# swesterfeld/audiowmark

Hardware: AMD Instinct MI355X
Metric: audio seconds watermarked+decoded per wall-second (xRT), 44.1 kHz stereo (higher is better)
Workload: dtype f32; 1 GPU; 60 min stereo 44.1 kHz white noise per GPU resident in HBM, add+get incl. payload decode, payload 0123456789abcdef0011223344556677, strength 10; parallelism=1 GPU, patterns=108, payload_matches=104, ranks_seen=1

## Files before the change

audiowmark_amd/csrc/hip/kernels.hip:

```cpp
#include "kernels.hh"
#include "awm_fft.hip.h"
#include <cstdlib>
#include <algorithm>
#include <type_traits>

namespace awmk {

constexpr int NB = 81;
constexpr int MIN_BAND = 20;
constexpr int WAVES = 4;

typedef const int __attribute__ ((address_space (4))) *const_int_ptr;

__device__ __forceinline__ void
load_shared_tables (const DevTables& t, float2 *s_tw, float *s_win, float2 *s_twb)
{
  fft512_load_twiddles (t.tw512, s_tw);
  for (int i = threadIdx.x; i < 1024; i += blockDim.x)
    s_win[i] = t.window[i];
  if (s_twb)
    for (int i = threadIdx.x; i < NB; i += blockDim.x)
      s_twb[i] = t.tw1024[MIN_BAND + i];
}

// ... 2900 lines not shown
  const int R = a.table.rows_per_bit;
  const_int_ptr tab = (const_int_ptr) (a.table.packed + (size_t) bit * R * 64);

  float umag = 0.f, dmag = 0.f;
  int n = 0;
  for (int r = 0; r < R; r++)
    {
      const_int_ptr tr = tab + r * 64;
      const long long row = tr[60];
      const bool present = have ? have[row * a.have_row_stride] != 0 : true;
      if (have && !__any (present))
        continue;
      const float *p = db + row * a.row_stride;
      float uv[30], dv[30];
#pragma unroll
      for (int i = 0; i < 30; i++)
        {
          uv[i] = p[tr[i] * a.band_stride];
          dv[i] = p[tr[30 + i] * a.band_stride];
        }
      if (present)
        {
#pragma unroll
          for (int i = 0; i < 30; i++)
            {
              umag = __fadd_rn (umag, uv[i]);
              dmag = __fadd_rn (dmag, dv[i]);
            }
          n++;
        }
    }
  s_u[bit][lane] = umag;
  s_d[bit][lane] = dmag;
  s_n[bit][lane] = n;
  __syncthreads();
  if (bit == 0 && active)
    {
      double q = 0;
      int total = 0;
      for (int b = 0; b < 6; b++)
        {
          const float um = s_u[b][lane], dm = s_d[b][lane];
          float raw;
          if (um == 0 || dm == 0)
            raw = 0;
          else if (um < dm)
            raw = __fsub_rn (1.f, __fdiv_rn (um, dm));
          else
            raw = __fsub_rn (__fdiv_rn (dm, um), 1.f);
          const double rb = (b & 1) ? double (raw) : -double (raw);
          q += rb * s_n[b][lane];
          total += s_n[b][lane];
        }
      if (total)
        q /= total;
      q = q / a.min_delta / 2.9;
      a.quality[plane * a.q_stride + cand] = q;
    }
}

hipError_t
launch_sync_scan (hipStream_t st, const SyncScanArgs& a)
{
  if (a.n_lanes <= 0 || a.n_planes <= 0)
    return hipSuccess;
  SyncScanArgs b = a;
  long long done = 0;
  while (done < a.n_planes)
    {
      const long long n = (a.n_planes - done) > 65535 ? 65535 : (a.n_planes - done);
      b.db = a.db + done * a.plane_stride;
      b.have = a.have ? a.have + done * a.have_plane_stride : nullptr;
      b.lane_count = a.lane_count ? a.lane_count + done : nullptr;
      b.quality = a.quality + done * a.q_stride;
      const long long per_xcd = ((a.n_lanes + 63) / 64 + 7) / 8;
      const dim3 grid (unsigned (per_xcd * 8), unsigned (n));
      hipLaunchKernelGGL (sync_scan_kernel, grid, dim3 (64, 6), 0, st, b);
      hipError_t e = hipGetLastError();
      if (e != hipSuccess)
        return e;
      done += n;
    }
  return hipSuccess;
}

template<bool HAVE> __global__ void __launch_bounds__ (64)
sync_scan_gathered_kernel (GatheredScanArgs a)
{
  const int lane = threadIdx.x;
  const long long plane = blockIdx.y;
  const int count = a.lane_count[plane];
  int chain, cand;
  if (int (blockIdx.x) < a.regular_waves)
    {
      chain = blockIdx.x % 12;
      cand = (blockIdx.x / 12) * 64 + lane;
    }
  else
    {
      chain = lane / a.tail_lanes;
      cand = a.tail_first + lane % a.tail_lanes;
    }
  const bool active = chain < 12 && cand < count;
  if (!__any (active))
    return;
  if (!active)
    chain = 0, cand = 0;
  const int bit = chain >> 1, down = chain & 1;
  const int R = a.rows_per_bit;
  const int ld = a.ld;
  const bool from_tail = a.tail && cand >= ld;
  const long long step = from_tail ? 1 : ld;
  const float *p = from_tail ? a.tail + plane * a.tail_plane_stride + ((long long) bit * R * 60 + down * 30)
                             : a.db + plane * a.plane_stride + ((long long) bit * R * 60 + down * 30) * ld + cand;
  const int hld = a.have_ld ? a.have_ld : ld;
  const char *hv = HAVE ? a.have + plane * a.have_plane_stride + (long long) bit * R * hld + cand : nullptr;

  float mag = 0.f;
  int n = 0;
  auto issue = [&] (int r, float (&v)[30], bool& present) {
    const float *q = p + (long long) r * 60 * step;
    present = HAVE ? hv[r * hld] != 0 : true;
    if (HAVE && !__any (present))
      return;
#pragma unroll
    for (int i = 0; i < 30; i++)
      v[i] = q[i * step];
  };
  auto accumulate = [&] (const float (&v)[30], bool present) {
    if (present)
      {
#pragma unroll
        for (int i = 0; i < 30; i++)
          mag = __fadd_rn (mag, v[i]);
        n++;
      }
  };
  float v[3][30];
  bool pr[3] = { false, false, false };
  const int last = R - 1;
  int r = 0;
  if (R > 0)
    {
#pragma unroll
      for (int k = 0; k < 2; k++)
        {
          issue (k < last ? k : last, v[k], pr[k]);
          __builtin_amdgcn_sched_barrier (0);
        }
      for (; r + 3 <= R; r += 3)
        {
#pragma unroll
          for (int k = 0; k < 3; k++)
            {
              const int nx = r + k + 2;
              issue (nx < last ? nx : last, v[(k + 2) % 3], pr[(k + 2) % 3]);
              __builtin_amdgcn_sched_barrier (0);
              accumulate (v[k], pr[k]);
              __builtin_amdgcn_sched_barrier (0);
            }
        }
#pragma unroll
      for (int k = 0; k < 2; k++)
        if (r + k < R)
          accumulate (v[k], pr[k]);
    }
  if (active)
    {
      a.chain_mag[(plane * 12 + chain) * 128 + cand] = mag;
      if (!down)
        a.chain_n[(plane * 6 + bit) * 128 + cand] = n;
    }
}

__global__ void __launch_bounds__ (64)
sync_quality_kernel (GatheredScanArgs a)
{
  const long long plane = blockIdx.y;
  const int cand = blockIdx.x * 64 + threadIdx.x;
  if (cand >= a.lane_count[plane])
    return;
  double q = 0;
  int total = 0;
  for (int b = 0; b < 6; b++)
    {
      const float um = a.chain_mag[(plane * 12 + 2 * b) * 128 + cand], dm = a.chain_mag[(plane * 12 + 2 * b + 1) * 128 + cand];
      const int n = a.chain_n[(plane * 6 + b) * 128 + cand];
      float raw;
      if (um == 0 || dm == 0)
        raw = 0;
      else if (um < dm)
        raw = __fsub_rn (1.f, __fdiv_rn (um, dm));
      else
        raw = __fsub_rn (__fdiv_rn (dm, um), 1.f);
      const double rb = (b & 1) ? double (raw) : -double (raw);
      q += rb * n;
      total += n;
    }
  if (total)
    q /= total;
  q = q / a.min_delta / 2.9;
  a.quality[plane * a.q_stride + cand] = q;
}

hipError_t
launch_sync_scan_gathered (hipStream_t st, const GatheredScanArgs& a0)
{
  if (a0.n_lanes <= 0 || a0.n_planes <= 0)
    return hipSuccess;
  if (!a0.lane_count || a0.n_planes > 65535 || a0.n_lanes > 128 || !a0.chain_mag || !a0.chain_n)
    return hipErrorInvalidValue;
  GatheredScanArgs a = a0;
  const int full = a.n_lanes / 64, rem = a.n_lanes % 64;
  const bool tail = rem > 0 && rem * 12 <= 64;
  a.regular_waves = 12 * (tail || rem == 0 ? full : full + 1);
  a.tail_first = 64 * full;
  a.tail_lanes = tail ? rem : 1;
  const dim3 grid (unsigned (a.regular_waves + (tail ? 1 : 0)), unsigned (a.n_planes));
  if (a.have)
    hipLaunchKernelGGL (sync_scan_gathered_kernel<true>, grid, dim3 (64), 0, st, a);
  else
    hipLaunchKernelGGL (sync_scan_gathered_kernel<false>, grid, dim3 (64), 0, st, a);
  hipLaunchKernelGGL (sync_quality_kernel, dim3 (unsigned ((a.n_lanes + 63) / 64), unsigned (a.n_planes)), dim3 (64), 0, st, a);
  return hipGetLastError();
}

__global__ void __launch_bounds__ (256)
local_mean_kernel (const double *q, long long q_stride, long long S, double *raw_sorted, double *local_mean)
{
  const long long p = (long long) blockIdx.x * blockDim.x + threadIdx.x;
  const long long n_scores = 4 * S;
  if (p >= n_scores)
    return;
  q += (long long) blockIdx.y * 4 * q_stride;
  raw_sorted += (long long) blockIdx.y * n_scores;
  local_mean += (long long) blockIdx.y * n_scores;
  double avg = 0;
  int n = 0;
  for (int j = -20; j <= 20; j++)
    {
      if (j > -4 && j < 4)
        continue;
      const long long idx = p + j;
      if (idx >= 0 && idx < n_scores)
        {
          avg += q[(idx & 3) * q_stride + (idx >> 2)];
          n++;
        }
    }
  if (n > 0)
    avg /= n;
  raw_sorted[p] = q[(p & 3) * q_stride + (p >> 2)];
  local_mean[p] = avg;
}

hipError_t
launch_local_mean (hipStream_t st, const double *q, long long q_stride, long long n_start_frames, double *raw_sorted, double *local_mean,
                   int n_slices)
{
  const long long n = 4 * n_start_frames;
  if (n <= 0 || n_slices <= 0)
    return hipSuccess;
  hipLaunchKernelGGL (local_mean_kernel, dim3 (unsigned ((n + 255) / 256), unsigned (n_slices)), dim3 (256), 0, st, q, q_stride, n_start_frames,
                      raw_sorted, local_mean);
  return hipGetLastError();
}

__global__ void __launch_bounds__ (128)
soft_bits_kernel (SoftBitsArgs a)
{
  const long long blk = blockIdx.y;
  const int bit = blockIdx.x * blockDim.x + threadIdx.x;
  const int n_bits = a.n_data_frames / a.frames_per_bit;
  if (bit >= n_bits)
    return;
  const float *db = a.db + blk * a.block_stride;
  const int C = a.n_channels;
  const long long mix0 = a.block_slice ? (long long) a.block_slice[blk] * a.n_data_frames * 30 : 0;
  const int16_t *mix_frame = a.mix_frame + mix0;
  const uint8_t *mix_up = a.mix_up + mix0, *mix_down = a.mix_down + mix0;
  double umag = 0, dmag = 0;
  for (int f = bit * a.frames_per_bit; f < (bit + 1) * a.frames_per_bit; f++)
    for (int ch = 0; ch < C; ch++)
      {
        const float *plane = db + (long long) ch * NB * a.ld;
        for (int j = 0; j < 30; j++)
          {
            const int b = f * 30 + j;
            const int frame = mix_frame[b];
            const int next = frame + 1 < a.block_frames ? frame + 1 : frame - 1;
            const int prev = frame - 1 >= 0 ? frame - 1 : frame + 1;
            const float *pu = plane + (long long) (mix_up[b] - MIN_BAND) * a.ld;
            const float *pd = plane + (long long) (mix_down[b] - MIN_BAND) * a.ld;
            umag += pu[frame];
            umag -= double (__fadd_rn (pu[prev], pu[next])) * 0.5;
            dmag += pd[frame];
            dmag -= double (__fadd_rn (pd[prev], pd[next])) * 0.5;
          }
      }
  a.out[blk * n_bits + bit] = float (umag - dmag);
}

constexpr int SB_WAVES = 4;
constexpr int SB_BPW = 4;
constexpr int SB_MAX_ITEMS = 256;

__global__ void __launch_bounds__ (64 * SB_WAVES)
soft_bits_wave_kernel (SoftBitsArgs a, int groups_per_block)
{
  extern __shared__ __attribute__ ((aligned (16))) float4 s_item_dyn[];
  const int lane = threadIdx.x & 63, wave = threadIdx.x >> 6;
  const long long slot = blockIdx.x >> 3;
  const long long blk = (slot / groups_per_block) * 8 + (blockIdx.x & 7);
  const int group = int (slot % groups_per_block);
  if (blk >= a.n_blocks)
    return;
  const int n_bits = a.n_data_frames / a.frames_per_bit;
  const int bit0 = (group * SB_WAVES + wave) * SB_BPW;
  if (bit0 >= n_bits)
    return;
  const float *db = a.db + blk * a.block_stride;
  const int C = a.n_channels;
  const long long mix0 = a.block_slice ? (long long) a.block_slice[blk] * a.n_data_frames * 30 : 0;
  const int16_t *mix_frame = a.mix_frame + mix0;
  const uint8_t *mix_up = a.mix_up + mix0, *mix_down = a.mix_down + mix0;
  const int n_items = a.frames_per_bit * C * 30;
  float4 *items = s_item_dyn + (size_t) wave * SB_BPW * n_items;
  const int n_here = min (SB_BPW, n_bits - bit0);
  int live_lo = 0, live_hi = 0x7fffffff;
  if (a.stream_range)
    {
      const long long sl = a.range_index[blk];
      const long long first = a.stream_range[2 * sl], last = a.stream_range[2 * sl + 1];
      live_lo = a.block_frames;
      live_hi = -1;
      if (first >= 0)
        {
          const long long base = a.block_base[blk];
          const long long lo_num = (first + C - 1) / C - 1024 - base, hi_num = last / C - base;
          const long long lo = lo_num <= 0 ? 0 : (lo_num + 1023) / 1024, hi = hi_num < 0 ? -1 : hi_num / 1024;
          live_lo = int (lo < a.block_frames ? lo : a.block_frames);
          live_hi = int (hi < a.block_frames ? hi : a.block_frames - 1);
        }
    }
  const float zero_db = db_from_complex (make_float2 (0.f, 0.f));
  for (int i = lane; i < n_items; i += 64)
#pragma unroll
  for (int q = 0; q < SB_BPW; q++)
    {
      const int e = q * n_items + i;
      const int bit = bit0 + min (q, n_here - 1);
      const int fi = i / (C * 30), ch = (i / 30) % C, j = i % 30;
      const int b = (bit * a.frames_per_bit + fi) * 30 + j;
      const int frame = mix_frame[b];
      const int next = frame + 1 < a.block_frames ? frame + 1 : frame - 1;
      const int prev = frame - 1 >= 0 ? frame - 1 : frame + 1;
      if (max (frame, max (prev, next)) < live_lo || min (frame, min (prev, next)) > live_hi)
        {
          items[e] = make_float4 (zero_db, __fadd_rn (zero_db, zero_db), zero_db, __fadd_rn (zero_db, zero_db));
          continue;
        }
      const float *plane = db + (long long) ch * NB * a.ld;
      const float *pu = plane + (long long) (mix_up[b] - MIN_BAND) * a.ld;
      const float *pd = plane + (long long) (mix_down[b] - MIN_BAND) * a.ld;
      items[e] = make_float4 (pu[frame], __fadd_rn (pu[prev], pu[next]), pd[frame], __fadd_rn (pd[prev], pd[next]));
    }
  wave_sync();
  if (lane < n_here)
    {
      const float4 *mine = items + lane * n_items;
      double umag = 0, dmag = 0;
      for (int i = 0; i < n_items; i++)
        {
          const float4 t = mine[i];
          umag = __dadd_rn (umag, double (t.x));
          umag = __dsub_rn (umag, __dmul_rn (double (t.y), 0.5));
          dmag = __dadd_rn (dmag, double (t.z));
          dmag = __dsub_rn (dmag, __dmul_rn (double (t.w), 0.5));
        }
      a.out[blk * n_bits + bit0 + lane] = float (__dsub_rn (umag, dmag));
    }
}

int g_soft_bits_generic = 0;
extern "C" void awm_debug_set_soft_bits_generic (int on) { g_soft_bits_generic = on; }

hipError_t
launch_soft_bits (hipStream_t st, const SoftBitsArgs& a)
{
  if (a.n_blocks <= 0)
    return hipSuccess;
  const int n_bits = a.n_data_frames / a.frames_per_bit;
  if (!g_soft_bits_generic && a.frames_per_bit * a.n_channels * 30 <= SB_MAX_ITEMS)
    {
      const int groups = (n_bits + SB_WAVES * SB_BPW - 1) / (SB_WAVES * SB_BPW);
      const long long rounds = (a.n_blocks + 7) / 8;
      const long long wgs = rounds * groups * 8;
      const size_t lds = size_t (SB_WAVES) * SB_BPW * (a.frames_per_bit * a.n_channels * 30) * sizeof (float4);
      if (wgs < (1LL << 31))
        {
          hipLaunchKernelGGL (soft_bits_wave_kernel, dim3 (unsigned (wgs)), dim3 (64 * SB_WAVES), lds, st, a, groups);
          return hipGetLastError();
        }
    }
  const dim3 grid (unsigned ((n_bits + 127) / 128), unsigned (a.n_blocks));
  hipLaunchKernelGGL (soft_bits_kernel, grid, dim3 (128), 0, st, a);
  return hipGetLastError();
}

__global__ void __launch_bounds__ (256)
nonzero_range_kernel (const float *data, long long n_values, unsigned long long *result)
{
  const long long stride = (long long) gridDim.x * blockDim.x;
  unsigned long long first = ~0ULL, last = 0;
  for (long long i = (long long) blockIdx.x * blockDim.x + threadIdx.x; i < n_values; i += stride)
    if (data[i] != 0.f)
      {
        if ((unsigned long long) i < first) first = i;
        if ((unsigned long long) i + 1 > last) last = i + 1;
      }
  for (int o = 32; o > 0; o >>= 1)
    {
      const unsigned long long f = __shfl_xor (first, o), l = __shfl_xor (last, o);
      first = f < first ? f : first;
      last = l > last ? l : last;
    }
  __shared__ unsigned long long s_first[4], s_last[4];
  if ((threadIdx.x & 63) == 0)
    {
      s_first[threadIdx.x >> 6] = first;
      s_last[threadIdx.x >> 6] = last;
    }
  __syncthreads();
  if (threadIdx.x == 0)
    {
      for (int w = 1; w < 4; w++)
        {
          first = s_first[w] < first ? s_first[w] : first;
          last = s_last[w] > last ? s_last[w] : last;
        }
      if (first != ~0ULL)
        {
          atomicMin (result, first);
          atomicMax (result + 1, last);
        }
    }
}

__global__ void __launch_bounds__ (256)
soft_prep_kernel (SoftPrepArgs a)
{
  __shared__ __attribute__ ((aligned (16))) float s_v[1728];
  __shared__ double s_mean;
  const SoftJobDev job = a.jobs[blockIdx.x];
  const int2 *src = a.src + job.src_off;
  const int nb = a.n_bits;
  const int *inv_order = a.inv_order + job.order_off;
  if (job.len > 1728)
    return;
  if (job.mode == 0)
    {
      const float *raw = a.raw + (long long) src[0].x * nb;
      for (int k = threadIdx.x; k < nb; k += 256)
        s_v[k] = raw[inv_order[k]];
    }
  else if (job.mode == 1)
    {
      for (int s = 0; s < job.n_src; s++)
        {
          const float *raw = a.raw + (long long) src[s].x * nb;
          const int half = src[s].y;
          for (int k = threadIdx.x; k < nb; k += 256)
            s_v[2 * k + half] = raw[inv_order[k]];
        }
    }
  else
    {
      const float div0 = float (job.norm0 > 1 ? job.norm0 : 1), div1 = float (job.norm1 > 1 ? job.norm1 : 1);
      for (int k = threadIdx.x; k < nb; k += 256)
        {
          const int i = inv_order[k];
          float acc0 = 0.f, acc1 = 0.f;
          int s = 0;
          for (; s + 8 <= job.n_src; s += 8)
            {
              float v[8];
              int half[8];
#pragma unroll
              for (int u = 0; u < 8; u++)
                {
                  const int2 sp = src[s + u];
                  v[u] = a.raw[(long long) sp.x * nb + i];
                  half[u] = sp.y;
                }
#pragma unroll
              for (int u = 0; u < 8; u++)
                {
                  if (half[u])
                    acc1 = __fadd_rn (acc1, v[u]);
                  else
                    acc0 = __fadd_rn (acc0, v[u]);
                }
            }
          for (; s < job.n_src; s++)
            {
              const float v = a.raw[(long long) src[s].x * nb + i];
              if (src[s].y)
                acc1 = __fadd_rn (acc1, v);
              else
                acc0 = __fadd_rn (acc0, v);
            }
          s_v[2 * k] = __fdiv_rn (acc0, div0);
          s_v[2 * k + 1] = __fdiv_rn (acc1, div1);
        }
    }
  __syncthreads();
  float *out = a.out + job.out_off;
  if (a.hard)
    {
      for (int k = threadIdx.x; k < job.len; k += 256)
        out[k] = s_v[k] > 0 ? 1.f : 0.f;
      return;
    }
  if (threadIdx.x == 0)
    {
      double mean = 0;
      int k = 0;
      for (; k + 32 <= job.len; k += 32)
        {
          float4 q[8];
#pragma unroll
          for (int i = 0; i < 8; i++)
            q[i] = reinterpret_cast<const float4 *> (s_v + k)[i];
#pragma unroll
          for (int i = 0; i < 8; i++)
            {
              mean = __dadd_rn (mean, double (fabsf (q[i].x)));
              mean = __dadd_rn (mean, double (fabsf (q[i].y)));
              mean = __dadd_rn (mean, double (fabsf (q[i].z)));
              mean = __dadd_rn (mean, double (fabsf (q[i].w)));
            }
        }
      for (; k < job.len; k++)
        mean = __dadd_rn (mean, double (fabsf (s_v[k])));
      s_mean = __ddiv_rn (mean, double (job.len));
    }
  __syncthreads();
  const double mean = s_mean;
  for (int k = threadIdx.x; k < job.len; k += 256)
    out[k] = float (__dmul_rn (0.5, __dadd_rn (__ddiv_rn (double (s_v[k]), mean), 1.0)));
}

hipError_t
launch_soft_prep (hipStream_t st, const SoftPrepArgs& a)
{
  if (a.n_jobs <= 0)
    return hipSuccess;
  hipLaunchKernelGGL (soft_prep_kernel, dim3 (unsigned (a.n_jobs)), dim3 (256), 0, st, a);
  return hipGetLastError();
}

hipError_t
launch_nonzero_range (hipStream_t st, const float *data, long long n_values, unsigned long long *result)
{
  hipError_t e = hipMemsetAsync (result, 0xff, sizeof (unsigned long long), st);
  if (e == hipSuccess)
    e = hipMemsetAsync (result + 1, 0, sizeof (unsigned long long), st);
  if (e != hipSuccess || n_values <= 0)
    return e;
  hipLaunchKernelGGL (nonzero_range_kernel, dim3 (1024), dim3 (256), 0, st, data, n_values, result);
  return hipGetLastError();
}

__global__ void __launch_bounds__ (256)
clip_pad_kernel (const ClipSrc *src, float *dst, long long slice_values, long long margin_values, unsigned long long *range)
{
  const ClipSrc c = src[blockIdx.y];
  float4 *out = reinterpret_cast<float4 *> (dst + (long long) blockIdx.y * slice_values);
  const long long slice0 = (long long) blockIdx.y * slice_values;
  const long long stride = (long long) gridDim.x * blockDim.x;
  unsigned long long first = ~0ULL, last = 0;
  long long q_lo = (c.pad_start - margin_values) / 4, q_hi = (c.pad_start + c.n_values + margin_values + 3) / 4;
  q_lo = q_lo < 0 ? 0 : q_lo;
  q_hi = q_hi > slice_values / 4 ? slice_values / 4 : q_hi;
  for (long long q = q_lo + (long long) blockIdx.x * blockDim.x + threadIdx.x; q < q_hi; q += stride)
    {
      const long long k = 4 * q - c.pad_start;
      float v[4] = { 0.f, 0.f, 0.f, 0.f };
      if (k > -4 && k < c.n_values)
        {
#pragma unroll
          for (int j = 0; j < 4; j++)
            if (k + j >= 0 && k + j < c.n_values)
              v[j] = c.data[k + j];
#pragma unroll
          for (int j = 0; j < 4; j++)
            if (v[j] != 0.f)
              {
                const unsigned long long at = (unsigned long long) (slice0 + 4 * q + j);
                first = at < first ? at : first;
                last = at + 1 > last ? at + 1 : last;
              }
        }
      out[q] = make_float4 (v[0], v[1], v[2], v[3]);
    }
  for (int o = 32; o > 0; o >>= 1)
    {
      const unsigned long long f = __shfl_xor (first, o), l = __shfl_xor (last, o);
      first = f < first ? f : first;
      last = l > last ? l : last;
    }
  __shared__ unsigned long long s_first[4], s_last[4];
  if ((threadIdx.x & 63) == 0)
    {
      s_first[threadIdx.x >> 6] = first;
      s_last[threadIdx.x >> 6] = last;
    }
  __syncthreads();
  if (threadIdx.x == 0)
    {
      for (int w = 1; w < 4; w++)
        {
          first = s_first[w] < first ? s_first[w] : first;
          last = s_last[w] > last ? s_last[w] : last;
        }
      if (first != ~0ULL)
        {
          atomicMin (range + 2 * blockIdx.y, first);
          atomicMax (range + 2 * blockIdx.y + 1, last);
        }
    }
}

__global__ void
clip_range_init_kernel (unsigned long long *range, int n_clips)
{
  const int i = blockIdx.x * blockDim.x + threadIdx.x;
  if (i < n_clips)
    {
      range[2 * i] = ~0ULL;
      range[2 * i + 1] = 0;
    }
}

int g_clip_poison = 0;
extern "C" void awm_debug_set_clip_poison (int on) { g_clip_poison = on; }

hipError_t
launch_clip_pad (hipStream_t st, const ClipSrc *src, int n_clips, float *dst, long long slice_values, long long margin_values, long long *range)
{
  if (n_clips <= 0 || slice_values <= 0)
    return hipSuccess;
  if (slice_values % 4 || margin_values < 0 || (reinterpret_cast<uintptr_t> (dst) & 15))
    return hipErrorInvalidValue;
  if (g_clip_poison)
    if (hipError_t e = hipMemsetAsync (dst, 0xff, size_t (n_clips) * size_t (slice_values) * sizeof (float), st))
      return e;
  auto *r = reinterpret_cast<unsigned long long *> (range);
  hipLaunchKernelGGL (clip_range_init_kernel, dim3 (unsigned ((n_clips + 255) / 256)), dim3 (256), 0, st, r, n_clips);
  hipLaunchKernelGGL (clip_pad_kernel, dim3 (128, unsigned (n_clips)), dim3 (256), 0, st, src, dst, slice_values, margin_values, r);
  return hipGetLastError();
}

constexpr int SEG_RUN = 2048;
__global__ void __launch_bounds__ (256)
segment_copy_kernel (const SegmentCopy *copies)
{
  const SegmentCopy c = copies[blockIdx.y];
  const long long n_zero = c.zeros / 2, n_total = n_zero + c.n_values / 2;
  const long long base = (long long) blockIdx.x * SEG_RUN;
  if (c.n_values <= 0 || base >= n_total)
    return;
  const float2 *src = reinterpret_cast<const float2 *> (c.src);
  float2 *dst = reinterpret_cast<float2 *> (c.dst);
  constexpr int U = SEG_RUN / 256;
  float2 v[U];
#pragma unroll
  for (int j = 0; j < U; j++)
    {
      const long long q = base + threadIdx.x + 256 * j;
      v[j] = q >= n_zero && q < n_total ? src[q - n_zero] : make_float2 (0.f, 0.f);
    }
#pragma unroll
  for (int j = 0; j < U; j++)
    {
      const long long q = base + threadIdx.x + 256 * j;
      if (q < n_total)
        dst[q] = v[j];
    }
}

hipError_t
launch_segment_copy (hipStream_t st, const SegmentCopy *copies_dev, int n_copies, long long max_values)
{
  if (n_copies <= 0 || max_values <= 0)
    return hipSuccess;
  const long long max_pieces = (max_values + 1) / 2;
  hipLaunchKernelGGL (segment_copy_kernel, dim3 (unsigned ((max_pieces + SEG_RUN - 1) / SEG_RUN), unsigned (n_copies)), dim3 (256), 0, st, copies_dev);
  return hipGetLastError();
}

// ... 355 lines not shown
```

Before: 748,700 xRT.

## Pipeline soft-bit gathers with wave-specialized double-buffered LDS slices

Restructures the soft-bits kernel so that one wave accumulates the double-precision sums for 16 bits while the other three waves gather the next frame/channel slice into a double-buffered, padded LDS tile. The gather loads a contiguous 3-float run per band, replacing three scalar loads, and batches several gathers per iteration to raise memory-level parallelism. It also shrinks LDS from a per-wave item array to two small slices, which may raise occupancy. In exchange it adds a block-wide barrier per slice and serialises the accumulation onto a single wave, so throughput depends on whether the gather or the FP64 accumulation dominates.

```diff
diff --git a/audiowmark_amd/csrc/hip/kernels.hip b/audiowmark_amd/csrc/hip/kernels.hip
--- a/audiowmark_amd/csrc/hip/kernels.hip
+++ b/audiowmark_amd/csrc/hip/kernels.hip
@@ -3226,8 +3226,13 @@
 }
 
 constexpr int SB_WAVES = 4;
-constexpr int SB_BPW = 4;
+constexpr int SB_BITS = 16;
+constexpr int SB_ROW = SB_BITS + 1;
+constexpr int SB_GATHER_DEPTH = 3;
 constexpr int SB_MAX_ITEMS = 256;
+
+typedef float SbRun __attribute__ ((ext_vector_type (3), aligned (4)));
+static __device__ __forceinline__ float sb_pick (SbRun r, int i) { return i == 0 ? r.x : i == 1 ? r.y : r.z; }
 
 __global__ void __launch_bounds__ (64 * SB_WAVES)
 soft_bits_wave_kernel (SoftBitsArgs a, int groups_per_block)
@@ -3240,17 +3245,13 @@
   if (blk >= a.n_blocks)
     return;
   const int n_bits = a.n_data_frames / a.frames_per_bit;
-  const int bit0 = (group * SB_WAVES + wave) * SB_BPW;
-  if (bit0 >= n_bits)
-    return;
+  const int bit0 = group * SB_BITS;
+  const int n_here = min (SB_BITS, n_bits - bit0);
   const float *db = a.db + blk * a.block_stride;
   const int C = a.n_channels;
   const long long mix0 = a.block_slice ? (long long) a.block_slice[blk] * a.n_data_frames * 30 : 0;
   const int16_t *mix_frame = a.mix_frame + mix0;
   const uint8_t *mix_up = a.mix_up + mix0, *mix_down = a.mix_down + mix0;
-  const int n_items = a.frames_per_bit * C * 30;
-  float4 *items = s_item_dyn + (size_t) wave * SB_BPW * n_items;
-  const int n_here = min (SB_BPW, n_bits - bit0);
   int live_lo = 0, live_hi = 0x7fffffff;
   if (a.stream_range)
     {
@@ -3268,42 +3269,85 @@
         }
     }
   const float zero_db = db_from_complex (make_float2 (0.f, 0.f));
-  for (int i = lane; i < n_items; i += 64)
-#pragma unroll
-  for (int q = 0; q < SB_BPW; q++)
-    {
-      const int e = q * n_items + i;
-      const int bit = bit0 + min (q, n_here - 1);
-      const int fi = i / (C * 30), ch = (i / 30) % C, j = i % 30;
-      const int b = (bit * a.frames_per_bit + fi) * 30 + j;
-      const int frame = mix_frame[b];
-      const int next = frame + 1 < a.block_frames ? frame + 1 : frame - 1;
-      const int prev = frame - 1 >= 0 ? frame - 1 : frame + 1;
-      if (max (frame, max (prev, next)) < live_lo || min (frame, min (prev, next)) > live_hi)
-        {
-          items[e] = make_float4 (zero_db, __fadd_rn (zero_db, zero_db), zero_db, __fadd_rn (zero_db, zero_db));
-          continue;
-        }
-      const float *plane = db + (long long) ch * NB * a.ld;
-      const float *pu = plane + (long long) (mix_up[b] - MIN_BAND) * a.ld;
-      const float *pd = plane + (long long) (mix_down[b] - MIN_BAND) * a.ld;
-      items[e] = make_float4 (pu[frame], __fadd_rn (pu[prev], pu[next]), pd[frame], __fadd_rn (pd[prev], pd[next]));
-    }
-  wave_sync();
-  if (lane < n_here)
-    {
-      const float4 *mine = items + lane * n_items;
-      double umag = 0, dmag = 0;
-      for (int i = 0; i < n_items; i++)
-        {
-          const float4 t = mine[i];
-          umag = __dadd_rn (umag, double (t.x));
-          umag = __dsub_rn (umag, __dmul_rn (double (t.y), 0.5));
-          dmag = __dadd_rn (dmag, double (t.z));
-          dmag = __dsub_rn (dmag, __dmul_rn (double (t.w), 0.5));
-        }
-      a.out[blk * n_bits + bit0 + lane] = float (__dsub_rn (umag, dmag));
-    }
+  const int n_slices = a.frames_per_bit * C;
+  const int n_terms = n_here * 30;
+
+  auto gather = [&] (int s, int first, int step)
+    {
+      float4 *buf = s_item_dyn + (s & 1) * (30 * SB_ROW);
+      const int fi = s / C;
+      const float *plane = db + (long long) (s % C) * NB * a.ld;
+      const int ld = int (a.ld);
+      for (; first < n_terms; first += SB_GATHER_DEPTH * step)
+        {
+          int frame[SB_GATHER_DEPTH], up[SB_GATHER_DEPTH], down[SB_GATHER_DEPTH], at[SB_GATHER_DEPTH];
+#pragma unroll
+          for (int u = 0; u < SB_GATHER_DEPTH; u++)
+            {
+              const int i = min (first + u * step, n_terms - 1);
+              const int q = i / 30, j = i - q * 30;
+              const int b = ((bit0 + q) * a.frames_per_bit + fi) * 30 + j;
+              frame[u] = mix_frame[b];
+              up[u] = mix_up[b];
+              down[u] = mix_down[b];
+              at[u] = j * SB_ROW + q;
+            }
+          SbRun ru[SB_GATHER_DEPTH], rd[SB_GATHER_DEPTH];
+          int i0[SB_GATHER_DEPTH], ip[SB_GATHER_DEPTH], in[SB_GATHER_DEPTH];
+          bool silent[SB_GATHER_DEPTH];
+#pragma unroll
+          for (int u = 0; u < SB_GATHER_DEPTH; u++)
+            {
+              const int next = frame[u] + 1 < a.block_frames ? frame[u] + 1 : frame[u] - 1;
+              const int prev = frame[u] - 1 >= 0 ? frame[u] - 1 : frame[u] + 1;
+              silent[u] = max (frame[u], max (prev, next)) < live_lo || min (frame[u], min (prev, next)) > live_hi;
+              const int live = silent[u] ? 0 : -1;
+              const int lo = min (max (frame[u] - 1, 0), a.block_frames - 3) & live;
+              ru[u] = *reinterpret_cast<const SbRun *> (plane + ((up[u] - MIN_BAND) * ld & live) + lo);
+              rd[u] = *reinterpret_cast<const SbRun *> (plane + ((down[u] - MIN_BAND) * ld & live) + lo);
+              i0[u] = (frame[u] & live) - lo;
+              ip[u] = (prev & live) - lo;
+              in[u] = (next & live) - lo;
+            }
+#pragma unroll
+          for (int u = 0; u < SB_GATHER_DEPTH; u++)
+            asm volatile ("" : "+v" (ru[u]), "+v" (rd[u]));
+#pragma unroll
+          for (int u = 0; u < SB_GATHER_DEPTH; u++)
+            if (first + u * step < n_terms)
+              buf[at[u]] = silent[u] ? make_float4 (zero_db, __fadd_rn (zero_db, zero_db), zero_db, __fadd_rn (zero_db, zero_db))
+                                     : make_float4 (sb_pick (ru[u], i0[u]), __fadd_rn (sb_pick (ru[u], ip[u]), sb_pick (ru[u], in[u])),
+                                                    sb_pick (rd[u], i0[u]), __fadd_rn (sb_pick (rd[u], ip[u]), sb_pick (rd[u], in[u])));
+        }
+    };
+
+  gather (0, threadIdx.x, 64 * SB_WAVES);
+  __syncthreads();
+  double umag = 0, dmag = 0;
+  for (int s = 0; s < n_slices; s++)
+    {
+      if (wave == 0)
+        {
+          if (lane < n_here)
+            {
+              const float4 *mine = s_item_dyn + (s & 1) * (30 * SB_ROW) + lane;
+#pragma unroll 10
+              for (int j = 0; j < 30; j++)
+                {
+                  const float4 t = mine[j * SB_ROW];
+                  umag = __dadd_rn (umag, double (t.x));
+                  umag = __dsub_rn (umag, __dmul_rn (double (t.y), 0.5));
+                  dmag = __dadd_rn (dmag, double (t.z));
+                  dmag = __dsub_rn (dmag, __dmul_rn (double (t.w), 0.5));
+                }
+            }
+        }
+      else if (s + 1 < n_slices)
+        gather (s + 1, threadIdx.x - 64, 64 * (SB_WAVES - 1));
+      __syncthreads();
+    }
+  if (wave == 0 && lane < n_here)
+    a.out[blk * n_bits + bit0 + lane] = float (__dsub_rn (umag, dmag));
 }
 
 int g_soft_bits_generic = 0;
@@ -3317,10 +3361,10 @@
   const int n_bits = a.n_data_frames / a.frames_per_bit;
   if (!g_soft_bits_generic && a.frames_per_bit * a.n_channels * 30 <= SB_MAX_ITEMS)
     {
-      const int groups = (n_bits + SB_WAVES * SB_BPW - 1) / (SB_WAVES * SB_BPW);
+      const int groups = (n_bits + SB_BITS - 1) / SB_BITS;
       const long long rounds = (a.n_blocks + 7) / 8;
       const long long wgs = rounds * groups * 8;
-      const size_t lds = size_t (SB_WAVES) * SB_BPW * (a.frames_per_bit * a.n_channels * 30) * sizeof (float4);
+      const size_t lds = size_t (2) * 30 * SB_ROW * sizeof (float4);
       if (wgs < (1LL << 31))
         {
           hipLaunchKernelGGL (soft_bits_wave_kernel, dim3 (unsigned (wgs)), dim3 (64 * SB_WAVES), lds, st, a, groups);
```

After: 754,400 xRT (median of 6 runs). About the same (+0.8%).
